# USCbiostats/fmcmc

Hardware: AMD Instinct MI355X
Metric: MH samples/sec (chains x iters / s), 1024 chains, 5-param linreg n=10k (higher is better)
Workload: dtype f64

## Files before the change

### fmcmc_amd/csrc/mh_mfma.hpp

```cpp
#pragma once
#include "mh_owner.hpp"

namespace {

constexpr int MF_NMF = 80;
constexpr int MF_TCS = 8 * PIPE_TRS + 2;

template <int KIND, int NG, int NS, bool DBG, bool BIG = false, bool EXT = false>
__global__ __launch_bounds__(NT) void mh_sweep_mfma(const SweepArgs A) {
  constexpr int CW = 4;
#ifndef MFO_MB
#define MFO_MB 12
#endif
  constexpr int MB = MFO_MB;
  constexpr int TN = NS * 4;
  static_assert(NG * TN <= MF_NMF, "operand registers");
  extern __shared__ double smem[];
  const int tid = threadIdx.x, lane = tid & 63;
  const int wave = __builtin_amdgcn_readfirstlane(tid >> 6);
  const int k = A.k, kz = A.kz;
  double* s_th1 = smem;
  double* s_par = s_th1 + CW * PIPE_KMAX;
  double* s_fold = s_par + 4 * PIPE_KMAX;
  const long long cg0 = (long long)blockIdx.x * CW;
  const int ncw = (int)((A.nchains - cg0 < CW) ? (A.nchains - cg0) : CW);
  const int nsteps = (int)A.nsteps, burnin = (int)A.burnin, thin = (int)A.thin;
  const int ic = A.intercept;

  const int feat = lane >> 4, o16 = lane & 15;
  const int cl_a = 16 * (o16 & 3) + 4 * (o16 >> 2);
  const int P = A.p;
  double areg[NG][TN];
#pragma unroll
  for (int q = 0; q < NG; q++) {
    const int f = 4 * q + feat;
#pragma unroll
    for (int t = 0; t < TN; t++) {
      const int sl = t >> 2, g = t & 3;
      const long long i = (long long)(64 * wave + cl_a + g) + (long long)NT * sl;
      double a = 0.0;
      if (i < A.n) {
        if (f < P) a = A.X[(long long)f * A.n + i];
        else if (f == P) a = A.y[i];
      }
      areg[q][t] = a;
    }
  }
  const int jch = lane & 3;
  const int cl_d = 16 * (lane >> 4) + 4 * ((lane >> 2) & 3);
  unsigned vbits = 0;
#pragma unroll
  for (int g = 0; g < 4; g++) {
    const int l = 64 * wave + cl_d + g;
    if ((long long)l + (long long)NT * (NS - 1 + (EXT ? A.mf_next : 0)) < A.n) vbits |= 1u << g;
  }
  if (tid < k) {
    s_par[0 * PIPE_KMAX + tid] = A.mu[tid];
    s_par[1 * PIPE_KMAX + tid] = A.scale[tid];
    s_par[2 * PIPE_KMAX + tid] = A.lb[tid];
    s_par[3 * PIPE_KMAX + tid] = A.ub[tid];
  }
  if (tid < CW * PIPE_KMAX) {
    const int c = tid / PIPE_KMAX, j = tid - c * PIPE_KMAX;
    s_th1[tid] = (c < ncw && j < k) ? A.theta0[(cg0 + c) * k + j] : 0.0;
  }

  const int myc = wave;
  const bool owner = (myc < ncw);
  const int cl = __builtin_amdgcn_readfirstlane((int)cg0 + (owner ? myc : 0));
  const bool plane = owner && (lane < k);
  const int jl = (lane < k) ? lane : 0;
  const bool fixed_l = A.fixed[jl] != 0;
  int zidx = 0;
  for (int j = 0; j < jl; j++) zidx += A.fixed[j] ? 0 : 1;
  if (zidx > kz - 1) zidx = kz > 0 ? kz - 1 : 0;
  double th0 = plane ? A.theta0[(long long)cl * k + lane] : 0.0;
  double th1 = th0;
  double f0 = 0.0;
  int nacc = 0;
  int status = (A.win_cont && owner) ? A.status[cl] : FMCMC_CHAIN_OK, thin_ctr = A.thin_ctr0;
  unsigned int bitword = 0;
  char* const s_base = reinterpret_cast<char*>(A.samples) + (BIG ? ((long long)cl * k) * A.ldS * 8 : 0ll);
  char* const d_base = A.draws ? reinterpret_cast<char*>(A.draws) + (BIG ? ((long long)cl * k) * A.ldS * 8 : 0ll) : nullptr;
  char* const l_base = A.logpost ? reinterpret_cast<char*>(A.logpost) + (BIG ? (long long)cl * A.ldS * 8 : 0ll) : nullptr;
  const unsigned int lane_off = (unsigned int)(((BIG ? 0ll : (long long)cl * k) + jl) * A.ldS * 8);
  const unsigned int lp_off = BIG ? 0u : (unsigned int)((long long)cl * A.ldS * 8);
  unsigned int srow8 = 0;
  const char* const z_base = reinterpret_cast<const char*>(A.fed_z) + (BIG ? ((long long)cl * nsteps) * kz * 8 : 0ll);
  const unsigned int z_lane = (unsigned int)(((BIG ? 0ll : (long long)cl * nsteps) * kz + zidx) * 8);
  const double* const lu_row = A.fed_logu + (long long)cl * nsteps;
  const double dn = uniform_d((double)A.n);
  auto ld_z = [&](int row) -> double {
    return *reinterpret_cast<const double*>(z_base + (z_lane + (unsigned int)row * (unsigned int)(kz * 8)));
  };
  const double mu_l = A.mu[jl], sc_l = A.scale[jl];
  double z_nx = (owner && kz > 0) ? ld_z(nsteps >= 2 ? 1 : 0) : 0.0;
  double lu_nx = owner ? lu_row[nsteps >= 2 ? 1 : 0] : 0.0;
  auto flush_bits = [&](int i) {
    if (A.accept_bits && lane == 0) {
      unsigned int* w = A.accept_bits + ((long long)cl * A.bits_stride + ((i - 1) >> 5));
      *w = (A.win_cont && i <= 32) ? (*w | bitword) : bitword;
    }
    bitword = 0;
  };
  lds_barrier();

  constexpr bool dbg = DBG;
  bool st_keep = false;
  bool st_acc = false;
  double st_th0 = 0.0, st_th1 = 0.0, st_f1 = 0.0;
  unsigned long long te = 0, tb1 = 0, to = 0, tb2 = 0, tf = 0, tc = 0, td = 0;
  for (int v = 1; v <= nsteps; v++) {
    unsigned long long t_0 = dbg ? clk() : 0;
    {
      const double* tj = s_th1 + jch * PIPE_KMAX;
      double bop[NG];
#pragma unroll
      for (int q = 0; q < NG; q++) {
        const int f = 4 * q + feat;
        bop[q] = (f < P) ? tj[ic + f] : (f == P ? -1.0 : 0.0);
      }
      const double cop = ic ? tj[0] : 0.0;
      double acc[4] = {0.0, 0.0, 0.0, 0.0};
      typedef double mf_d4 __attribute__((ext_vector_type(4)));
      constexpr int RD = (NG == 1) ? 4 : 2;
      const int next = EXT ? A.mf_next : 0;
      const mf_d4* sp = reinterpret_cast<const mf_d4*>(A.mf_stream) + ((long long)wave * next * NG) * 64 + lane;
      mf_d4 ring[EXT ? RD : 1][NG];
      if constexpr (EXT) {
        const int rlast = next > 0 ? next - 1 : 0;
#pragma unroll
        for (int r = 0; r < RD; r++)
#pragma unroll
          for (int q = 0; q < NG; q++) ring[r][q] = sp[(((r < next) ? r : rlast) * NG + q) * 64];
      }
#pragma unroll
      for (int t0 = 0; t0 < TN; t0 += MB) {
        {
          constexpr int LAST = TN - 4;
          const int nu = (TN - t0 < MB) ? TN - t0 : MB;
          double d[MB];
#pragma unroll
          for (int u = 0; u < MB; u++)
            if (u < nu) {
              const int t = t0 + u;
              const double cm = ((!EXT || next == 0) && t >= LAST) ? (((vbits >> (t - LAST)) & 1u) ? cop : 0.0) : cop;
              d[u] = __builtin_amdgcn_mfma_f64_4x4x4f64(areg[0][t], bop[0], cm, 0, 0, 0);
            }
#pragma unroll
          for (int q = 1; q < NG; q++)
#pragma unroll
            for (int u = 0; u < MB; u++)
              if (u < nu) d[u] = __builtin_amdgcn_mfma_f64_4x4x4f64(areg[q][t0 + u], bop[q], d[u], 0, 0, 0);
#pragma unroll
          for (int u = 0; u < MB; u++)
            if (u < nu) acc[u & 3] = fmh_fma(d[u], d[u], acc[u & 3]);
        }
      }
      if constexpr (EXT) {
        double cml[4];
#pragma unroll
        for (int g = 0; g < 4; g++) cml[g] = ((vbits >> g) & 1u) ? cop : 0.0;
        for (int e0 = 0; e0 < next; e0 += RD) {
#pragma unroll
          for (int r = 0; r < RD; r++) {
            const int e = e0 + r;
            if (e < next) {
              mf_d4 a[NG];
#pragma unroll
              for (int q = 0; q < NG; q++) a[q] = ring[r][q];
              const int en = (e + RD < next) ? e + RD : next - 1;
#pragma unroll
              for (int q = 0; q < NG; q++) ring[r][q] = sp[(en * NG + q) * 64];
              const bool last = (e == next - 1);
              double d[4];
#pragma unroll
              for (int g = 0; g < 4; g++) d[g] = __builtin_amdgcn_mfma_f64_4x4x4f64(a[0][g], bop[0], last ? cml[g] : cop, 0, 0, 0);
#pragma unroll
              for (int q = 1; q < NG; q++)
#pragma unroll
                for (int g = 0; g < 4; g++) d[g] = __builtin_amdgcn_mfma_f64_4x4x4f64(a[q][g], bop[q], d[g], 0, 0, 0);
#pragma unroll
              for (int g = 0; g < 4; g++) acc[g] = fmh_fma(d[g], d[g], acc[g]);
            }
          }
        }
      }
      double fs = (acc[0] + acc[1]) + (acc[2] + acc[3]);
      fs = fs + dpp_d<0x114>(fs);
      fs = fs + dpp_d<0x118>(fs);
      {
        const unsigned long long u = (unsigned long long)__double_as_longlong(fs);
        const unsigned lo = (unsigned)u, hi = (unsigned)(u >> 32);
        const auto rl = __builtin_amdgcn_permlane16_swap(lo, lo, false, false);
        const auto rh = __builtin_amdgcn_permlane16_swap(hi, hi, false, false);
        fs = __longlong_as_double((long long)(((unsigned long long)rh[0] << 32) | rl[0])) +
             __longlong_as_double((long long)(((unsigned long long)rh[1] << 32) | rl[1]));
      }
      {
        const unsigned long long u = (unsigned long long)__double_as_longlong(fs);
        const unsigned lo = (unsigned)u, hi = (unsigned)(u >> 32);
        const auto rl = __builtin_amdgcn_permlane32_swap(lo, lo, false, false);
        const auto rh = __builtin_amdgcn_permlane32_swap(hi, hi, false, false);
        fs = __longlong_as_double((long long)(((unsigned long long)rh[0] << 32) | rl[0])) +
             __longlong_as_double((long long)(((unsigned long long)rh[1] << 32) | rl[1]));
      }
      if (lane >= 60) s_fold[jch * NW + wave] = fs;
    }
    double sigma = 0.0, nt1_fast = 0.0, ss_fast = 1.0, rs_fast = 1.0;
    bool sg_fast = false, ok_fast = false;
    if (owner) {
      sigma = readlane_d(th1, k - 1);
      const unsigned sg_hi = (unsigned)(fmh_d2u(sigma) >> 32);
      sg_fast = (sg_hi - 0x00100000u) < 0x7fe00000u;
      const double sg = sg_fast ? sigma : 1.0;
#ifdef MFO_NOLOG
      const double t1_fast = sg + FMH_K(FMH_LN_SQRT_2PI);
#else
      const double t1_fast = fmh_log_pn(sg) + FMH_K(FMH_LN_SQRT_2PI);
#endif
      nt1_fast = uniform_d(dn * t1_fast);
      ss_fast = uniform_d(sg * sg);
      ok_fast = sg_fast && mfr_div_safe(ss_fast);
      rs_fast = uniform_d(div_recip(ok_fast ? ss_fast : 1.0));
    }
    unsigned long long t_1 = dbg ? clk() : 0;
    lds_barrier();
    unsigned long long t_2 = dbg ? clk() : 0;
    if (owner) {
      __builtin_amdgcn_s_setprio(3);
      double wsum = s_fold[myc * NW + (lane & 7)];
      double lu = lu_nx, zc = z_nx;
      asm volatile("" : "+v"(lu), "+v"(zc));
      const double dz = mu_l + sc_l * zc;
      wsum = wsum + dpp_d<0xB1>(wsum);
      wsum = wsum + dpp_d<0x4E>(wsum);
      const double tot = wsum + dpp_d<0x141>(wsum);
      unsigned long long t_a = dbg ? clk() : 0;
      const double h = 0.5 * tot;
      double f1 = -nt1_fast - div_finish(h, ss_fast, rs_fast);
      unsigned long long t_b = dbg ? clk() : 0;
      const double th1_eval = th1;
      bool keep_row = true, acc = false;
      const double ratio_f = f1 - f0;
      const bool rare = (v == 1) || (status != FMCMC_CHAIN_OK) || !ok_fast || !mfr_div_safe(h) || fmh_isnan(ratio_f);
      auto propose = [&](bool frozen) {
        double t = th0 + dz;
        if (KIND == FMCMC_KERNEL_NORMAL_REFLECTIVE) {
          if (plane && !fixed_l) t = reflect1(t, s_par[2 * PIPE_KMAX + lane], s_par[3 * PIPE_KMAX + lane]);
        }
        t = fixed_l ? th0 : t;
        th1 = frozen ? th1 : t;
        if (plane) s_th1[myc * PIPE_KMAX + lane] = th1;
      };
      double th0_row;
      if (__builtin_expect(!__any(rare), 1)) {
        acc = lu < ratio_f;
        th0 = acc ? th1 : th0;
        f0 = acc ? f1 : f0;
        th0_row = th0;
        propose(false);
      } else {
        keep_row = false;
        if (sg_fast) {
          f1 = -nt1_fast - h / ss_fast;
          if (A.guard && !fmh_isfinite(f1)) f1 = -fmh_inf();
        } else {
          f1 = linreg_logpost(tot, sigma, dn, A.guard);
        }
        if (v == 1) {
          f0 = f1;
          keep_row = true;
        } else if (status == FMCMC_CHAIN_OK) {
          const double ratio = f1 - f0;
          if (fmh_isnan(f1) || fmh_isnan(ratio)) {
            status = fmh_isnan(f1) ? FMCMC_CHAIN_NAN_LOGPOST : FMCMC_CHAIN_NAN_RATIO;
            if (lane == 0) { A.status[cl] = status; A.status_step[cl] = v + A.step_off; }
            if (plane) A.status_theta[(long long)cl * k + lane] = th1;
            flush_bits(v);
          } else {
            acc = lu < ratio;
            keep_row = true;
          }
        }
        th0 = acc ? th1 : th0;
        f0 = acc ? f1 : f0;
        th0_row = th0;
        propose(status != FMCMC_CHAIN_OK);
      }
      st_acc = acc;
      unsigned long long t_c = dbg ? clk() : 0;
      if (dbg) { tf += t_a - t_2; tc += t_b - t_a; td += t_c - t_b; }
      __builtin_amdgcn_s_setprio(0);
      st_keep = keep_row; st_th0 = th0_row; st_th1 = th1_eval; st_f1 = f1;
    }
    unsigned long long t_3 = dbg ? clk() : 0;
    lds_barrier();
    if (dbg) { unsigned long long t_4 = clk(); te += t_1 - t_0; tb1 += t_2 - t_1; to += t_3 - t_2; tb2 += t_4 - t_3; }
    if (owner) {
      lu_nx = lu_row[v < nsteps ? v : nsteps - 1];
      if (kz > 0) z_nx = ld_z(v + 1 < nsteps ? v + 1 : nsteps - 1);
      nacc += st_acc ? 1 : 0;
      bitword |= (st_acc ? 1u : 0u) << ((v - 1) & 31);
      if (st_keep && v > burnin) {
        thin_ctr += 1;
        if (thin_ctr == thin) {
          thin_ctr = 0;
          if (plane) {
            *reinterpret_cast<double*>(s_base + (lane_off + srow8)) = st_th0;
            if (d_base) *reinterpret_cast<double*>(d_base + (lane_off + srow8)) = st_th1;
          }
          if (l_base && lane == 0 && !dbg) *reinterpret_cast<double*>(l_base + (lp_off + srow8)) = st_f1;
          srow8 += 8;
        }
      }
      if (status == FMCMC_CHAIN_OK && v >= 2 && (((v - 1) & 31) == 31 || v == nsteps)) flush_bits(v);
    }
  }
  if (dbg && lane == 0 && A.logpost) {
    double* d = A.logpost + (long long)A.nchains * A.S - 8 * ((long long)blockIdx.x * NW + wave + 1);
    d[0] = (double)te; d[1] = (double)tb1; d[2] = (double)to; d[3] = (double)tb2; d[4] = (double)nsteps; d[5] = (double)tf; d[6] = (double)tc; d[7] = (double)td;
  }
  if (owner) {
    if (plane) A.theta0[(long long)cl * k + lane] = th0;
    if (lane == 0) {
      A.f0[cl] = f0;
      A.accept_count[cl] = nacc;
      if (status == FMCMC_CHAIN_OK) { A.status[cl] = FMCMC_CHAIN_OK; A.status_step[cl] = 0; }
    }
  }
}

size_t mfma_lds_bytes() { return sizeof(double) * ((size_t)8 * PIPE_KMAX + 4 * NW); }

}
```

Baseline: 498.8 million.

## Precompute sigma-dependent logpost terms over a speculative accept/reject tree

For the plain normal kernel with a single operand group, each owner wave speculatively enumerates sigma proposals for the next five accept/reject outcomes, one tree node per lane. For each node it precomputes log(sigma), sigma squared and its reciprocal into an LDS table. Each step then walks the tree by the accept bit and reads the entry instead of doing a log and a divide on the critical serial path. This adds a rebuild every six steps or after a rare-path event, extra LDS space, clamped lookahead loads of z, and a noinline build call.

Result: faster. 507.9 million, median of 6 (+1.8%).

```diff
diff --git a/fmcmc_amd/csrc/mh_mfma.hpp b/fmcmc_amd/csrc/mh_mfma.hpp
--- a/fmcmc_amd/csrc/mh_mfma.hpp
+++ b/fmcmc_amd/csrc/mh_mfma.hpp
@@ -1,5 +1,6 @@
 #pragma once
 #include "mh_owner.hpp"
+#include "mh_sigtree.hpp"
 
 namespace {
 
@@ -9,6 +10,7 @@
 template <int KIND, int NG, int NS, bool DBG, bool BIG = false, bool EXT = false>
 __global__ __launch_bounds__(NT) void mh_sweep_mfma(const SweepArgs A) {
   constexpr int CW = 4;
+  constexpr bool TREE = KIND == FMCMC_KERNEL_NORMAL && NG == 1 && !BIG && !EXT;
 #ifndef MFO_MB
 #define MFO_MB 12
 #endif
@@ -22,6 +24,7 @@
   double* s_th1 = smem;
   double* s_par = s_th1 + CW * PIPE_KMAX;
   double* s_fold = s_par + 4 * PIPE_KMAX;
+  double* s_tree = s_fold + CW * NW;
   const long long cg0 = (long long)blockIdx.x * CW;
   const int ncw = (int)((A.nchains - cg0 < CW) ? (A.nchains - cg0) : CW);
   const int nsteps = (int)A.nsteps, burnin = (int)A.burnin, thin = (int)A.thin;
@@ -71,8 +74,10 @@
   const bool plane = owner && (lane < k);
   const int jl = (lane < k) ? lane : 0;
   const bool fixed_l = A.fixed[jl] != 0;
+  const int look = lane - ST_ZLANE;
+  const bool zl = TREE && look >= 0 && look < ST_LOOK;
   int zidx = 0;
-  for (int j = 0; j < jl; j++) zidx += A.fixed[j] ? 0 : 1;
+  for (int j = 0; j < (zl ? k - 1 : jl); j++) zidx += A.fixed[j] ? 0 : 1;
   if (zidx > kz - 1) zidx = kz > 0 ? kz - 1 : 0;
   double th0 = plane ? A.theta0[(long long)cl * k + lane] : 0.0;
   double th1 = th0;
@@ -87,11 +92,13 @@
   const unsigned int lp_off = BIG ? 0u : (unsigned int)((long long)cl * A.ldS * 8);
   unsigned int srow8 = 0;
   const char* const z_base = reinterpret_cast<const char*>(A.fed_z) + (BIG ? ((long long)cl * nsteps) * kz * 8 : 0ll);
-  const unsigned int z_lane = (unsigned int)(((BIG ? 0ll : (long long)cl * nsteps) * kz + zidx) * 8);
+  const unsigned int z_lane = (unsigned int)((((BIG ? 0ll : (long long)cl * nsteps) + (zl ? look : 0)) * kz + zidx) * 8);
+  const unsigned int z_end = (unsigned int)((((BIG ? 0ll : (long long)cl * nsteps) + nsteps) * kz - 1) * 8);
   const double* const lu_row = A.fed_logu + (long long)cl * nsteps;
   const double dn = uniform_d((double)A.n);
   auto ld_z = [&](int row) -> double {
-    return *reinterpret_cast<const double*>(z_base + (z_lane + (unsigned int)row * (unsigned int)(kz * 8)));
+    const unsigned int off = z_lane + (unsigned int)row * (unsigned int)(kz * 8);
+    return *reinterpret_cast<const double*>(z_base + ((!TREE || off < z_end) ? off : z_end));
   };
   const double mu_l = A.mu[jl], sc_l = A.scale[jl];
   double z_nx = (owner && kz > 0) ? ld_z(nsteps >= 2 ? 1 : 0) : 0.0;
@@ -110,6 +117,18 @@
   bool st_acc = false;
   double st_th0 = 0.0, st_th1 = 0.0, st_f1 = 0.0;
   unsigned long long te = 0, tb1 = 0, to = 0, tb2 = 0, tf = 0, tc = 0, td = 0;
+  int node = ST_NODES;
+  double nt1_fast = 0.0, ss_fast = 1.0, rs_fast = 1.0;
+  int st_fl = 0;
+  auto look_up = [&]() {
+    typedef double st_d2 __attribute__((ext_vector_type(2)));
+    const st_d2* e = reinterpret_cast<const st_d2*>(s_tree + myc * ST_TAB + node * ST_ENTRY);
+    const st_d2 e0 = e[0], e1 = e[1];
+    nt1_fast = uniform_d(e0[0]);
+    ss_fast = uniform_d(e0[1]);
+    rs_fast = uniform_d(e1[0]);
+    st_fl = __builtin_amdgcn_readfirstlane((int)__double_as_longlong(e1[1]));
+  };
   for (int v = 1; v <= nsteps; v++) {
     unsigned long long t_0 = dbg ? clk() : 0;
     {
@@ -207,22 +226,33 @@
       }
       if (lane >= 60) s_fold[jch * NW + wave] = fs;
     }
-    double sigma = 0.0, nt1_fast = 0.0, ss_fast = 1.0, rs_fast = 1.0;
+    double sigma = 0.0;
     bool sg_fast = false, ok_fast = false;
-    if (owner) {
-      sigma = readlane_d(th1, k - 1);
-      const unsigned sg_hi = (unsigned)(fmh_d2u(sigma) >> 32);
-      sg_fast = (sg_hi - 0x00100000u) < 0x7fe00000u;
-      const double sg = sg_fast ? sigma : 1.0;
+    if constexpr (TREE) {
+      if (owner && node >= ST_NODES) {
+        sigtree_build<KIND>((st_lds_d*)(s_tree + myc * ST_TAB), (const st_lds_d*)s_par, th0, th1, z_nx, k, (int)((__ballot(fixed_l) >> (k - 1)) & 1ull), dn);
+        node = 0;
+        look_up();
+      }
+      sg_fast = (st_fl & 1) != 0;
+      ok_fast = (st_fl & 2) != 0;
+    } else {
+      nt1_fast = 0.0; ss_fast = 1.0; rs_fast = 1.0;
+      if (owner) {
+        sigma = readlane_d(th1, k - 1);
+        const unsigned sg_hi = (unsigned)(fmh_d2u(sigma) >> 32);
+        sg_fast = (sg_hi - 0x00100000u) < 0x7fe00000u;
+        const double sg = sg_fast ? sigma : 1.0;
 #ifdef MFO_NOLOG
-      const double t1_fast = sg + FMH_K(FMH_LN_SQRT_2PI);
+        const double t1_fast = sg + FMH_K(FMH_LN_SQRT_2PI);
 #else
-      const double t1_fast = fmh_log_pn(sg) + FMH_K(FMH_LN_SQRT_2PI);
+        const double t1_fast = fmh_log_pn(sg) + FMH_K(FMH_LN_SQRT_2PI);
 #endif
-      nt1_fast = uniform_d(dn * t1_fast);
-      ss_fast = uniform_d(sg * sg);
-      ok_fast = sg_fast && mfr_div_safe(ss_fast);
-      rs_fast = uniform_d(div_recip(ok_fast ? ss_fast : 1.0));
+        nt1_fast = uniform_d(dn * t1_fast);
+        ss_fast = uniform_d(sg * sg);
+        ok_fast = sg_fast && mfr_div_safe(ss_fast);
+        rs_fast = uniform_d(div_recip(ok_fast ? ss_fast : 1.0));
+      }
     }
     unsigned long long t_1 = dbg ? clk() : 0;
     lds_barrier();
@@ -261,12 +291,13 @@
         th0_row = th0;
         propose(false);
       } else {
+        if constexpr (TREE) node = ST_STALE;
         keep_row = false;
         if (sg_fast) {
           f1 = -nt1_fast - h / ss_fast;
           if (A.guard && !fmh_isfinite(f1)) f1 = -fmh_inf();
         } else {
-          f1 = linreg_logpost(tot, sigma, dn, A.guard);
+          f1 = linreg_logpost(tot, TREE ? readlane_d(th1_eval, k - 1) : sigma, dn, A.guard);
         }
         if (v == 1) {
           f0 = f1;
@@ -301,6 +332,10 @@
       lu_nx = lu_row[v < nsteps ? v : nsteps - 1];
       if (kz > 0) z_nx = ld_z(v + 1 < nsteps ? v + 1 : nsteps - 1);
       nacc += st_acc ? 1 : 0;
+      if constexpr (TREE) {
+        node = st_child(node, __builtin_amdgcn_readfirstlane(st_acc ? 1 : 0));
+        if (node < ST_NODES) look_up();
+      }
       bitword |= (st_acc ? 1u : 0u) << ((v - 1) & 31);
       if (st_keep && v > burnin) {
         thin_ctr += 1;
@@ -331,6 +366,6 @@
   }
 }
 
-size_t mfma_lds_bytes() { return sizeof(double) * ((size_t)8 * PIPE_KMAX + 4 * NW); }
+size_t mfma_lds_bytes() { return sizeof(double) * ((size_t)8 * PIPE_KMAX + 4 * NW + 4 * ST_TAB); }
 
 }
diff --git a/fmcmc_amd/csrc/mh_sigtree.hpp b/fmcmc_amd/csrc/mh_sigtree.hpp
--- /dev/null
+++ b/fmcmc_amd/csrc/mh_sigtree.hpp
@@ -0,0 +1,69 @@
+#pragma once
+
+namespace {
+
+constexpr int ST_DEPTH = 6;
+constexpr int ST_NODES = (1 << ST_DEPTH) - 1;
+constexpr int ST_LOOK = ST_DEPTH - 1;
+constexpr int ST_ZLANE = 32;
+constexpr int ST_ENTRY = 4;
+constexpr int ST_TAB = 64 * ST_ENTRY;
+constexpr int ST_STALE = ST_NODES / 2;
+
+constexpr int st_depth(int node) { int d = 0; while ((2 << d) - 1 <= node) d++; return d; }
+constexpr int st_path(int node) { return node + 1 - (1 << st_depth(node)); }
+constexpr int st_child(int node, int accept) { return 2 * node + 1 + accept; }
+constexpr bool st_consistent() {
+  for (int i = 0; i < ST_NODES; i++) {
+    if (st_depth(i) >= ST_DEPTH || st_path(i) >> st_depth(i)) return false;
+    for (int a = 0; a < 2; a++) {
+      const int c = st_child(i, a);
+      if (st_depth(c) != st_depth(i) + 1 || st_path(c) != 2 * st_path(i) + a) return false;
+      if ((st_depth(i) == ST_DEPTH - 1) != (c >= ST_NODES)) return false;
+    }
+  }
+  return st_depth(0) == 0 && st_child(ST_STALE, 0) >= ST_NODES && ST_ZLANE + ST_LOOK <= 64;
+}
+static_assert(st_consistent(), "tree indices");
+
+typedef __attribute__((address_space(3))) double st_lds_d;
+template <int KIND>
+__device__ __noinline__ void sigtree_build(st_lds_d* tab, const st_lds_d* par, double th0, double th1, double z, int k, int fixed, double dn) {
+  const int lane = threadIdx.x & 63;
+  const int d = 31 - __builtin_clz(lane + 1), path = lane + 1 - (1 << d);
+  const double mu = par[0 * PIPE_KMAX + k - 1], sc = par[1 * PIPE_KMAX + k - 1];
+  const double lb = par[2 * PIPE_KMAX + k - 1], ub = par[3 * PIPE_KMAX + k - 1];
+  double a = readlane_d(th0, k - 1), b = readlane_d(th1, k - 1);
+#pragma unroll 1
+  for (int j = 0; j < ST_LOOK; j++) {
+    const bool on = j < d;
+    const double dz = mu + sc * readlane_d(z, ST_ZLANE + j);
+    const bool acc = ((path >> (on ? d - 1 - j : 0)) & 1) != 0;
+    const double a1 = acc ? b : a;
+    double t = a1 + dz;
+    if (KIND == FMCMC_KERNEL_NORMAL_REFLECTIVE) {
+      if (on && !fixed) t = reflect1(t, lb, ub);
+    }
+    t = fixed ? a1 : t;
+    a = on ? a1 : a;
+    b = on ? t : b;
+  }
+  const unsigned sg_hi = (unsigned)(fmh_d2u(b) >> 32);
+  const bool sg_fast = (sg_hi - 0x00100000u) < 0x7fe00000u;
+  const double sg = sg_fast ? b : 1.0;
+#ifdef MFO_NOLOG
+  const double t1 = sg + FMH_K(FMH_LN_SQRT_2PI);
+#else
+  const double t1 = fmh_log_pn(sg) + FMH_K(FMH_LN_SQRT_2PI);
+#endif
+  const double ss = sg * sg;
+  const bool ok = sg_fast && mfr_div_safe(ss);
+  const double rs = div_recip(ok ? ss : 1.0);
+  typedef double st_d2 __attribute__((ext_vector_type(2)));
+  typedef __attribute__((address_space(3))) st_d2 st_lds_d2;
+  st_lds_d2* e = (st_lds_d2*)(tab + lane * ST_ENTRY);
+  e[0] = st_d2{dn * t1, ss};
+  e[1] = st_d2{rs, __longlong_as_double((long long)((sg_fast ? 1 : 0) | (ok ? 2 : 0)))};
+}
+
+}
```
